# nemochina2008/soundgen_beta

Hardware: AMD Instinct MI355X
Metric: synthesized audio samples/sec (whole node) @44.1 kHz; RMS error vs R ref (higher is better)
Workload: dtype fp32 (fp64 phase)

## Files before the change

soundgen_beta_amd/csrc/sg_dev.h:

```cpp
#pragma once
#include <stdint.h>

struct SgSeg {
  double t0;
  double c0, c1, c2, c3, c4;
};

struct SgEpoch {
  int64_t w_off;
  int64_t amp_off;
  int64_t knot_off;
  int32_t seg_off;
  int32_t nseg;
  int32_t n;
  int32_t G;
  int32_t R;
  int32_t u0;
  double x1, xG;
  double xby;
  double invD;
  int32_t dj0, dj1;
  int64_t dk0;
  int32_t syl;
  int32_t pad;
// ... 125 lines not shown
  int32_t pad;
  int64_t chirp;
  int64_t bf;
};
struct SgFftGeom {
  SgCdft cd[2];
  int32_t wl, M, nstages, fb;
  int32_t radix[SG_FFT_MAX_STAGES];
  int64_t tw;
  int64_t win;
  int32_t lds_bytes;
  int32_t kind;
  uint32_t mr_magic[SG_FFT_MAX_STAGES], ns_magic[SG_FFT_MAX_STAGES];
  uint32_t m_magic, hp_magic;
  int64_t tws;
};

constexpr int SG_FFT_WG = 0;
constexpr int SG_FFT_WAVE = 1;
constexpr int SG_FFT_DFT = 2;
constexpr int SG_FFT_ODD = 3;
constexpr int SG_WAVE_STATE = 24;
constexpr int SG_FFT_WAVES = 8;

#ifndef SG_NOISE_WAVES
#define SG_NOISE_WAVES 12
#endif
constexpr int SG_FFT_WAVES_NOISE = SG_NOISE_WAVES;
constexpr int sg_fft_waves(int phase) { return phase == 0 ? SG_FFT_WAVES_NOISE : SG_FFT_WAVES; }
constexpr int SG_PF_SRC = 20;
constexpr int SG_PF_PAIR = 10;
// ... 161 lines not shown
```

soundgen_beta_amd/csrc/sg_exec.cpp:

```cpp
#include "sg_exec.h"
#include "sg_amp.h"
#include "sg_prof.h"

#include <algorithm>
#include <chrono>
#include <exception>
#include <thread>
#include <cmath>
#include <climits>
#include <atomic>
#include <map>
#include <cstdlib>
#include <cstdio>
#include <cstring>
#include <string>

namespace sg {

namespace {
#define HIPCHK(x)                                                                         \
  do {                                                                                    \
    hipError_t _e = (x);                                                                  \
    if (_e != hipSuccess)                                                                 \
      throw SgError(SG_E_DEVICE, std::string(#x) + ": " + hipGetErrorString(_e));     \
// ... 784 lines not shown
  DevicePlan& D0 = *runs[0].D;
  HIPCHK(hipEventRecord(D0.ev_fork, s));
  HIPCHK(hipStreamWaitEvent(s2, D0.ev_fork, 0));
  for (const PlanRun& r : runs) {
    device_execute_harm(*r.B, *r.D, r.out, s2, nullptr);
    HIPCHK(hipEventRecord(r.D->ev_join, s2));
  }
  for (const PlanRun& r : runs) device_execute_spec(*r.B, *r.D, r.out, s, nullptr, true, r.D->ev_join);
  HIPCHK(hipGetLastError());
}

void device_execute_spec(const Batch& B, const DevicePlan& D, float* d_out, hipStream_t s,
                         std::vector<SgProfEvent>* prof, bool join, hipEvent_t harm_done) {
  launch_spec_env(D, B, s);
  auto phase = [&](int ph) {
    const int64_t* r = B.fgroup_range[ph];
    const int64_t nseg = B.seg_range[ph][1] - B.seg_range[ph][0];
    hipEvent_t e0 = nullptr, e1 = nullptr;
    if (prof && nseg > 0) {
      HIPCHK(hipEventCreate(&e0));
      HIPCHK(hipEventCreate(&e1));
      HIPCHK(hipEventRecord(e0, s));
    }
    launch_stft_ola(D, ph, B.seg_range[ph][0], nseg, B.fgroup_lds[ph][0], s);
    if (prof && nseg > 0) {
      HIPCHK(hipEventRecord(e1, s));
      prof->push_back({SG_PROF_STFT_OLA, e0, e1});
    }
    launch_fft_frames(D, r[1], r[2] - r[1], B.fgroup_lds[ph][1], s);
    launch_fft_frames64(D, B, ph, s);
    const int64_t t0 = ph == 0 ? 0 : B.olatile_split, t1 = ph == 0 ? B.olatile_split : (int64_t)B.olatiles.size();
    const int64_t o0 = ph == 0 ? 0 : B.ola_split, o1 = ph == 0 ? B.ola_split : (int64_t)B.olas_dev.size();
    launch_ola(D, t0, t1 - t0, s);
    launch_ola_max(D, o0, o1 - o0, s);
  };
  phase(0);
  for (const Batch::Copy& c : B.copies)
    HIPCHK(hipMemcpyAsync(D.fs + c.fs_off, D.fl + c.fl_off, (size_t)c.n * sizeof(float), hipMemcpyDeviceToDevice, s));
  if (join) HIPCHK(hipStreamWaitEvent(s, harm_done, 0));
  launch_mix(D, 0, B.mixtile_hp, d_out, s);
  launch_mix_hp(D, B.mixtile_hp, B.mixtile_split - B.mixtile_hp, s);
  phase(1);
  launch_mix(D, B.mixtile_split, (int64_t)B.mixtiles.size() - B.mixtile_split, d_out, s);
  HIPCHK(hipGetLastError());
// ... 4 lines not shown
```

soundgen_beta_amd/csrc/sg_exec.h:

```cpp
#pragma once
#include <hip/hip_runtime.h>

#include <utility>
#include <vector>

#include "sg_plan.h"

namespace sg {

struct PcmJob {
  char* buf = nullptr;
  SgPcmCall* calls = nullptr;
  SgPcmTile* tiles = nullptr;
  SgPcmStat* stats = nullptr;
  int64_t n = 0, ntiles = 0;
  void prepare(const int64_t* off, const int64_t* len, int64_t n_calls, hipStream_t s);
  void run(const void* in, bool f64, int mode, double nrange, int16_t* out, hipStream_t s) const;
  void free();
};

struct DevicePlan {
  bool uploaded = false;
  char* arena = nullptr;
  size_t arena_bytes = 0;
// ... 88 lines not shown
void launch_ugather(const SgUJob* jobs, int64_t n_jobs, const float* us, float* fl, hipStream_t s);
void launch_sine_bank(const DevicePlan& D, int64_t k0, int64_t n, hipStream_t s);
void launch_sine_bank_pairs(const DevicePlan& D, int64_t k0, int64_t n, hipStream_t s);
void launch_sine_bank_tall(const DevicePlan& D, int64_t k0, int64_t n, hipStream_t s);
void launch_sine_bank_tall_pairs(const DevicePlan& D, int64_t k0, int64_t n, hipStream_t s);
void launch_syl_max(const DevicePlan& D, int64_t s0, int64_t n_syls, hipStream_t s);
void launch_piece_max(const DevicePlan& D, int64_t p0, int64_t n_ptiles, hipStream_t s);
void launch_harm_finalize(const DevicePlan& D, int64_t f0, int64_t n_stiles, float* out, hipStream_t s);
void launch_harm_copy(const DevicePlan& D, int64_t c0, int64_t n_ctiles, float* out, hipStream_t s);
void launch_sine_bank_hp(const DevicePlan& D, int64_t n, hipStream_t s);
void launch_sine_bank_tab(const DevicePlan& D, int logn, int64_t j0, int64_t n, float* out, hipStream_t s);
void launch_piece_max_hp(const DevicePlan& D, int64_t p0, int64_t n_ptiles, hipStream_t s);
void launch_harm_finalize_hp(const DevicePlan& D, int64_t n_stiles, hipStream_t s);
void launch_mix_hp(const DevicePlan& D, int64_t t0, int64_t n_tiles, hipStream_t s);
void launch_fft_frames64(const DevicePlan& D, const Batch& B, int ph, hipStream_t s);
void launch_fft_frames(const DevicePlan& D, int64_t g0, int64_t n_groups, int lds_bytes, hipStream_t s);
void launch_stft_ola(const DevicePlan& D, int phase, int64_t s0, int64_t n_segs, int lds_bytes, hipStream_t s);
void launch_ola(const DevicePlan& D, int64_t t0, int64_t n_tiles, hipStream_t s);
void launch_ola_max(const DevicePlan& D, int64_t o0, int64_t n_olas, hipStream_t s);
void launch_fft_probe(const SgFftGeom* geom, const float* fl, float* data, int M, int nframes, int inverse,
                      hipStream_t s);
void launch_mix(const DevicePlan& D, int64_t t0, int64_t n_tiles, float* out, hipStream_t s);
void launch_spec_env(const DevicePlan& D, const Batch& B, hipStream_t s);

}
```

soundgen_beta_amd/csrc/sg_fft.hip:

```cpp
#include <hip/hip_runtime.h>

#include <type_traits>

#include "sg_dev.h"
#include "sg_devfn.h"
#include "sg_fft64_dev.h"
#include "sg_roots.h"

namespace {

typedef float v2 __attribute__((ext_vector_type(2)));
__device__ __forceinline__ v2 V(float2 a) { return v2{a.x, a.y}; }
__device__ __forceinline__ float2 F(v2 a) { return make_float2(a.x, a.y); }
__device__ __forceinline__ v2 pfma(v2 a, v2 b, v2 c) { return __builtin_elementwise_fma(a, b, c); }
__device__ __forceinline__ v2 splat(float c) { return v2{c, c}; }
__device__ __forceinline__ v2 vmul(v2 a, v2 w) {
  v2 t, r;
  __asm__("v_pk_mul_f32 %0, %1, %2 op_sel_hi:[0,1]" : "=v"(t) : "v"(a), "v"(w));
  __asm__("v_pk_fma_f32 %0, %1, %2, %3 op_sel:[1,1,0] op_sel_hi:[1,0,1] neg_lo:[0,1,0]"
          : "=v"(r) : "v"(a), "v"(w), "v"(t));
  return r;
}
__device__ __forceinline__ v2 vmulc(v2 a, v2 w) {
  v2 t, r;
// ... 92 lines not shown

__device__ __forceinline__ void pack_pair(float2 yk, float2 ymk, float2 wNk, float2& zk, float2& zmk) {
  const float2 e = cadd(yk, cconj(ymk));
  const float2 d = csub(yk, cconj(ymk));
  const float2 o = cmulc(d, wNk);
  zk = make_float2(e.x - o.y, e.y + o.x);
  const float2 e2 = cadd(ymk, cconj(yk));
  const float2 d2 = csub(ymk, cconj(yk));
  const float2 o2 = make_float2(-(d2.x * wNk.x - d2.y * wNk.y), -(d2.x * wNk.y + d2.y * wNk.x));
  zmk = make_float2(e2.x - o2.y, e2.y + o2.x);
}

constexpr int SG_FFT_THREADS = 512;
constexpr int SG_FFT_SLOTS = 8192;

template <int R>
struct NbOf {
  static constexpr int value = (SG_FFT_SLOTS / SG_FFT_THREADS + R - 1) / R;
};

__device__ __forceinline__ int udiv(int n, uint32_t magic) {
  return magic ? (int)__umulhi((uint32_t)n, magic) : n;
}

template <int R, bool INV>
__device__ __forceinline__ void stage_ip(float2* X, int M, int Ns, const float2* twS, int fb, uint32_t mr_magic,
                                         uint32_t ns_magic) {
  constexpr int NB = NbOf<R>::value;
  constexpr bool ODD = (R % 2) == 1;
  constexpr int H = ODD ? (R - 1) / 2 : 1;
  const int MR = M / R;
  const int total = fb * MR;
  v2 st[NB][R];
  int base_o[NB];
  bool live[NB];
#pragma unroll
  for (int q = 0; q < NB; ++q) {
    const int idx = threadIdx.x + q * SG_FFT_THREADS;
    live[q] = idx < total;
    base_o[q] = 0;
    if (!live[q]) continue;
    const int f = udiv(idx, mr_magic);
    const int j = idx - f * MR;
    const float2* x = X + f * M;
    float2 v[R];
#pragma unroll
    for (int r = 0; r < R; ++r) v[r] = x[j + r * MR];
    const int jm = j - udiv(j, ns_magic) * Ns;
    if (Ns > 1) {
      const float2* tw = twS + (Ns - 1) + jm;
#pragma unroll
      for (int r = 1; r < R; ++r) {
        const float2 w = tw[(r - 1) * Ns];
// ... 27 lines not shown
#pragma unroll
      for (int k = 1; k <= H; ++k) {
        v2 a, b;
        odd_out<R, INV>(st[q], k, a, b);
        y[k * Ns] = F(a);
        y[(R - k) * Ns] = F(b);
      }
    } else {
#pragma unroll
      for (int r = 0; r < R; ++r) y[r * Ns] = F(st[q][r]);
    }
  }
  __syncthreads();
}

template <bool INV>
__device__ void fft_ip(float2* X, const SgFftGeom& g, const float2* twS, int fb) {
  int Ns = 1;
  for (int s = 0; s < g.nstages; ++s) {
    const int R = g.radix[s];
    const uint32_t mm = g.mr_magic[s], nm = g.ns_magic[s];
    int Ms = g.M;
    Ms = __builtin_amdgcn_readfirstlane(Ms);
    switch (R) {
#define SG_STAGE(RR) \
      case RR: stage_ip<RR, INV>(X, Ms, Ns, twS, fb, mm, nm); break;
      SG_STAGE(2) SG_STAGE(3) SG_STAGE(4) SG_STAGE(5) SG_STAGE(7) SG_STAGE(11) SG_STAGE(13) SG_STAGE(17)
      SG_STAGE(19) SG_STAGE(23) SG_STAGE(29) SG_STAGE(31)
#undef SG_STAGE
      default: break;
    }
    Ns *= R;
  }
}

__device__ __forceinline__ void sg_wave_fence() { __asm__ __volatile__("" ::: "memory"); }

template <int R>
struct NbW {
  static constexpr int value = SG_WAVE_STATE / R > 0 ? SG_WAVE_STATE / R : 1;
};

#ifndef SG_R19_REMAP
#define SG_R19_REMAP 1
#endif
template <int R, bool INV, int CM = 0, int CNS = 0>
__device__ __forceinline__ void stage_w(float2* X, int M_, int Ns_, const float2* twS, uint32_t ns_magic, int lane) {
  constexpr int NB = NbW<R>::value;
// ... 220 lines not shown
  }
  sg_wave_fence();
}

template <bool INV, int CM, int R0, int R1, int R2, bool MFMA = true, bool LAST = true>
__device__ __forceinline__ void fft_wc(float2* X, const float2* twS, const float4* A29, int lane SG_ST_PARAMS) {
  if constexpr (MFMA && CM == 1102 && R0 == 29) stage29_mfma<INV>(X, A29, lane);
  else stage_w<R0, INV, CM, 1>(X, CM, 1, twS, 0u, lane);
  SG_ST(INV ? 5 : 1);
  stage_w<R1, INV, CM, R0>(X, CM, R0, twS, 0u, lane);
  SG_ST(INV ? 6 : 2);
  if constexpr (LAST) stage_w<R2, INV, CM, R0 * R1>(X, CM, R0 * R1, twS, 0u, lane);
  SG_ST(INV ? 7 : 3);
}

template <bool INV>
__device__ void cdft(float2* X, const SgCdft& c, const SgFftGeom* __restrict__ geoms, const float* __restrict__ fl,
                     float2* Z, float2* tw) {
  const SgFftGeom& gs = geoms[c.geom];
  const int T = c.L ? c.L : c.n;
  const float2* twg = reinterpret_cast<const float2*>(fl + gs.tws);
  for (int t = threadIdx.x; t < T - 1; t += SG_FFT_THREADS) tw[t] = twg[t];
  if (!c.L) {
    __syncthreads();
    fft_ip<INV>(X, gs, tw, 1);
    return;
  }
  const int n = c.n, L = c.L;
  const float2* ch = reinterpret_cast<const float2*>(fl + c.chirp);
  const float2* bf = reinterpret_cast<const float2*>(fl + c.bf);
  for (int j = threadIdx.x; j < L; j += SG_FFT_THREADS)
    Z[j] = j < n ? cmul(INV ? cconj(X[j]) : X[j], ch[j]) : make_float2(0.f, 0.f);
  __syncthreads();
  fft_ip<false>(Z, gs, tw, 1);
  for (int k = threadIdx.x; k < L; k += SG_FFT_THREADS) Z[k] = cmul(Z[k], bf[k]);
  __syncthreads();
  fft_ip<true>(Z, gs, tw, 1);
  for (int k = threadIdx.x; k < n; k += SG_FFT_THREADS) {
    const float2 v = cmul(Z[k], ch[k]);
    X[k] = INV ? cconj(v) : v;
  }
  __syncthreads();
}

__device__ void odd_frame(const SgFrameGroup& G, const SgFrame* __restrict__ frames, const SgFftGeom& g,
                          const SgFftGeom* __restrict__ geoms, const float* __restrict__ fl, float* __restrict__ fs,
                          float4* lds4) {
  const int N = g.wl, M = g.M, N2 = 2 * M;
  const int T = max(g.cd[0].L ? g.cd[0].L : g.cd[0].n, g.cd[1].L ? g.cd[1].L : g.cd[1].n);
  float2* B = reinterpret_cast<float2*>(lds4);
  float2* Z = B + N;
  float2* tw = Z + T;
  const SgFrame F = frames[G.f0];
  const float* ham = fl + g.win;
  const float* han = ham + N;
  if (G.mode == SG_FRAME_FILTER) {
    const float* s = fs + F.src;
    for (int n = threadIdx.x; n < N; n += SG_FFT_THREADS) B[n] = make_float2(s[n] * ham[n], 0.f);
    __syncthreads();
    cdft<false>(B, g.cd[0], geoms, fl, Z, tw);
    const float* env = fl + F.env;
    const float invN = 1.f / (float)N;
    for (int k = threadIdx.x; k < M; k += SG_FFT_THREADS) {
      const float sc = invN * env[k];
      const float2 y = make_float2(B[k].x * sc, B[k].y * sc);
      B[k] = y;
      if (k > 0) B[N2 - k] = cconj(y);
      if (k == M - 1) B[M] = make_float2(y.x, 0.f);
    }
  } else {
    const float* u = fl + F.src;
    const float* flt = fl + F.env;
    for (int k = threadIdx.x; k < M; k += SG_FFT_THREADS) {
      const float2 y = make_float2(u[k] * flt[k], 0.f);
      B[k] = y;
      if (k > 0) B[N2 - k] = y;
      if (k == M - 1) B[M] = y;
    }
  }
  __syncthreads();
  cdft<true>(B, g.cd[1], geoms, fl, Z, tw);
  const float invN2 = 1.f / (float)N2;
  float* d = fs + F.dst;
  for (int i = threadIdx.x; i < N; i += SG_FFT_THREADS) d[i] = B[i < N2 ? i : i - N2].x * invN2 * han[i];
}

}

extern "C" __global__ __launch_bounds__(SG_FFT_THREADS) void sg_fft_frames(
    const SgFrameGroup* __restrict__ groups, const SgFrame* __restrict__ frames, const SgFftGeom* __restrict__ geoms,
    const float* __restrict__ fl, float* __restrict__ fs) {
  extern __shared__ float4 lds4[];
  float2* A = reinterpret_cast<float2*>(lds4);
  __shared__ SgFrame fr[16];
  const SgFrameGroup G = groups[blockIdx.x];
  const SgFftGeom& g = geoms[G.geom];
  if (g.kind == SG_FFT_ODD) {
    odd_frame(G, frames, g, geoms, fl, fs, lds4);
    return;
  }
  const int M = g.M, N = g.wl, fb = G.nf;
  const float2* twg = reinterpret_cast<const float2*>(fl + g.tw);
  const float2* twN = twg + M;
  float2* twM = A + fb * M;
  if (g.kind != SG_FFT_DFT) {
    const float2* tsg = reinterpret_cast<const float2*>(fl + g.tws);
    for (int t = threadIdx.x; t < M - 1; t += SG_FFT_THREADS) twM[t] = tsg[t];
  }
  if (threadIdx.x < fb) fr[threadIdx.x] = frames[G.f0 + threadIdx.x];
  __syncthreads();
  const float* ham = fl + g.win;
  const float* han = ham + N;
  const float invN = 1.f / (float)N;
  const int half = M / 2;
  const int npairs = fb * (half + 1);
  constexpr int NP = SG_FFT_SLOTS / 2 / SG_FFT_THREADS + 1;
  if (G.mode == SG_FRAME_FILTER) {
    for (int idx = threadIdx.x; idx < fb * M; idx += SG_FFT_THREADS) {
      const int f = udiv(idx, g.m_magic), n = idx - f * M;
      const float* s = fs + fr[f].src;
      A[idx] = make_float2(s[2 * n] * ham[2 * n], s[2 * n + 1] * ham[2 * n + 1]);
    }
    __syncthreads();
    if (g.kind == SG_FFT_DFT) cdft<false>(A, g.cd[0], geoms, fl, twM, twM + g.cd[0].L);
    else fft_ip<false>(A, g, twM, fb);
    float2 zk[NP], zm[NP], zh[NP];
    int pk[NP], pf[NP];
#pragma unroll
    for (int q = 0; q < NP; ++q) {
      const int idx = threadIdx.x + q * SG_FFT_THREADS;
      pk[q] = -1;
      if (idx >= npairs) continue;
      const int f = udiv(idx, g.hp_magic), k = idx - f * (half + 1);
      if (k != 0 && k >= M - k) continue;
      pk[q] = k;
      pf[q] = f;
      const float2* z = A + f * M;
      const float* env = fl + fr[f].env;
      auto X_at = [&](int kk) -> float2 {
        const float2 a = z[kk], b = z[(M - kk) % M];
        const float2 e = make_float2(0.5f * (a.x + b.x), 0.5f * (a.y - b.y));
        const float2 dd = make_float2(a.x - b.x, a.y + b.y);
        const float2 o = make_float2(0.5f * dd.y, -0.5f * dd.x);
        return cadd(e, cmul(o, twN[kk]));
      };
      if (k == 0) {
        const float2 x0 = X_at(0), xl = X_at(M - 1);
        const float y0 = x0.x * invN * env[0];
        const float nyq = xl.x * invN * env[M - 1];
        zk[q] = make_float2(y0 + nyq, y0 - nyq);
        if (M % 2 == 0) {
          const float2 xk = X_at(half);
          const float2 yk = make_float2(xk.x * invN * env[half], xk.y * invN * env[half]);
// ... 10 lines not shown
    __syncthreads();
#pragma unroll
    for (int q = 0; q < NP; ++q) {
      if (pk[q] < 0) continue;
      float2* out = A + pf[q] * M;
      const int k = pk[q];
      out[k] = zk[q];
      if (k == 0) {
        if (M % 2 == 0) out[half] = zh[q];
      } else {
        out[M - k] = zm[q];
      }
    }
    __syncthreads();
  } else {
    for (int idx = threadIdx.x; idx < npairs; idx += SG_FFT_THREADS) {
      const int f = udiv(idx, g.hp_magic), k = idx - f * (half + 1);
      const SgFrame& F = fr[f];
      const float* u = fl + F.src;
      const float* flt = fl + F.env;
      float2* out = A + f * M;
      if (k == 0) {
        const float y0 = u[0] * flt[0], nyq = u[M - 1] * flt[M - 1];
        out[0] = make_float2(y0 + nyq, y0 - nyq);
        if (M % 2 == 0) {
          const float2 yk = make_float2(u[half] * flt[half], 0.f);
          float2 a, b;
          pack_pair(yk, yk, twN[half], a, b);
          out[half] = a;
        }
      } else if (k < M - k) {
        const float2 yk = make_float2(u[k] * flt[k], 0.f), ym = make_float2(u[M - k] * flt[M - k], 0.f);
        float2 a, b;
        pack_pair(yk, ym, twN[k], a, b);
        out[k] = a;
        out[M - k] = b;
      }
    }
    __syncthreads();
  }
  if (g.kind == SG_FFT_DFT) cdft<true>(A, g.cd[0], geoms, fl, twM, twM + g.cd[0].L);
  else fft_ip<true>(A, g, twM, fb);
  for (int idx = threadIdx.x; idx < fb * M; idx += SG_FFT_THREADS) {
    const int f = udiv(idx, g.m_magic), n = idx - f * M;
    const float2 v = A[idx];
    float* d = fs + fr[f].dst;
    d[2 * n] = v.x * invN * han[2 * n];
    d[2 * n + 1] = v.y * invN * han[2 * n + 1];
  }
}

static_assert(SG_PF_PAIR <= SG_PF_SRC, "noise filter pairs alias the sound pairs");
struct FramePf {
  float2 s[SG_PF_SRC];
  float2 a[SG_PF_PAIR];
  float xh, xh2;
  __device__ __forceinline__ float2& b(int i) { return s[i]; }
  __device__ __forceinline__ const float2& b(int i) const { return s[i]; }
};

template <bool FUSED = false>
__device__ __forceinline__ void frame_prefetch(FramePf& P, const SgFrame& F, int mode, int M,
                                               const float* __restrict__ fl, const float* __restrict__ fs, int lane) {
  const int half = M / 2;
// ... 1037 lines not shown
  } while (0)

static void lds_opt_in(const void* fn, int lds_bytes, const char* name) {
  static std::mutex mu;
  static std::map<std::pair<const void*, int>, int> done;
  int dev = 0;
  if (hipGetDevice(&dev) != hipSuccess) throw SgError(SG_E_DEVICE, std::string(name) + ": hipGetDevice failed");
  std::lock_guard<std::mutex> lk(mu);
  int& have = done[{fn, dev}];
  if (lds_bytes <= have) return;
  if (hipFuncSetAttribute(fn, hipFuncAttributeMaxDynamicSharedMemorySize, lds_bytes) != hipSuccess)
    throw SgError(SG_E_DEVICE, std::string(name) + ": dynamic LDS " + std::to_string(lds_bytes) + " B refused");
  have = lds_bytes;
}

void launch_fft_frames(const DevicePlan& D, int64_t g0, int64_t n_groups, int lds_bytes, hipStream_t s) {
  if (n_groups <= 0) return;
  lds_opt_in(reinterpret_cast<const void*>(&sg_fft_frames), lds_bytes, "sg_fft_frames");
  hipLaunchKernelGGL(sg_fft_frames, dim3((unsigned)n_groups), dim3(SG_FFT_THREADS), lds_bytes, s, D.fgroups + g0,
                     D.frames,
                     D.geoms, D.fl, D.fs);
  SG_LAUNCHED("sg_fft_frames");
}
void launch_stft_ola(const DevicePlan& D, int phase, int64_t s0, int64_t n_segs, int lds_bytes, hipStream_t s) {
  if (n_segs <= 0) return;
  auto* k = phase == 0 ? &sg_stft_ola_noise : &sg_stft_ola;
  lds_opt_in(reinterpret_cast<const void*>(k), lds_bytes, phase == 0 ? "sg_stft_ola_noise" : "sg_stft_ola");
  const int W = sg_fft_waves(phase);
  if (n_segs % W) throw SgError(SG_E_DEVICE, "sg_stft_ola: segment count not a multiple of the workgroup's waves");
  hipLaunchKernelGGL(k, dim3((unsigned)(n_segs / W)), dim3(W * 64), lds_bytes, s,
                     D.olasegs + s0,
                     D.olas, D.frames, D.geoms, D.fl, D.fs, D.olatilemax);
  SG_LAUNCHED("sg_stft_ola");
}
void launch_fft_probe(const SgFftGeom* geom, const float* fl, float* data, int M, int nframes, int inverse,
                      hipStream_t s) {
// ... 70 lines not shown
```

soundgen_beta_amd/csrc/sg_plan.h:

```cpp
#pragma once
#include <cstdint>
#include <functional>
#include <memory>
#include <utility>
#include <vector>

#include "sg_dev.h"
#include "sg_rmath.h"
#include "soundgen_hip.h"

namespace sg {

template <class T>
struct NoInitAlloc : std::allocator<T> {
  template <class U>
  struct rebind { using other = NoInitAlloc<U>; };
  NoInitAlloc() = default;
  template <class U>
  NoInitAlloc(const NoInitAlloc<U>&) noexcept {}
  T* allocate(size_t n) {
    if (n * sizeof(T) < SG_BULK_HUGE) return std::allocator<T>::allocate(n);
    return static_cast<T*>(bulk_alloc(n * sizeof(T)));
  }
  void deallocate(T* p, size_t n) noexcept {
// ... 75 lines not shown
  std::vector<SgOla> olas[2];
  std::vector<SgFrame64> frames64;
  std::vector<int32_t> roots64_wl;
  std::vector<int64_t> roots64_off, frames64_tab;
  int64_t roots64_total = 0;
  int32_t frames64_maxwl = 0;
  int64_t frames64_noise = 0;
  int64_t frames64_w[2] = {0, 0};
  std::vector<SgNoiseItem> items;
  std::vector<SgMix> mixes[2];
  struct Copy { int64_t fl_off, fs_off, n; };
  std::vector<Copy> copies;
  std::vector<SgFrameGroup> fgroups;
  int64_t fgroup_range[2][3] = {{0, 0, 0}, {0, 0, 0}};
  int fgroup_lds[2][2] = {{0, 0}, {0, 0}};
  std::vector<SgOla> olas_dev;
  std::vector<SgOlaTile> olatiles;
  int64_t olatile_split = 0, ola_split = 0;
  std::vector<SgSegment> olasegs;
  int32_t n_segslots = 0;
  int64_t seg_range[2][2] = {{0, 0}, {0, 0}};
  std::vector<SgMix> mixes_dev;
  std::vector<SgMixTile> mixtiles;
  int64_t mixtile_split = 0;
  int64_t mixtile_hp = 0;
  bulk<double> cknots;
  int64_t w_total = 0;
  int64_t w64_total = 0;
  int64_t fh_total = 0;
  int64_t hp_bouts = 0;
// ... 91 lines not shown
```

soundgen_beta_amd/csrc/sg_plan_spec.cpp:

```cpp
#include <algorithm>
#include <atomic>
#include <cmath>
#include <complex>
#include <cstdio>
#include <cstdlib>
#include <cstring>
#include <map>
#include <memory>
#include <mutex>
#include <string>

#include "sg_plan.h"
#include "sg_prof.h"

#ifndef SG_SEG_SORT
#define SG_SEG_SORT 1
#endif
#ifndef SG_ENV_SORT
#define SG_ENV_SORT 1
#endif

namespace sg {

namespace {
// ... 115 lines not shown
      b[m] = std::complex<double>((*ch)[2 * m], -(*ch)[2 * m + 1]);
      if (m > 0) b[L - m] = b[m];
    }
    dft_smooth(b, bf);
    vec v(2 * (size_t)L);
    for (int k = 0; k < L; ++k) {
      v[2 * k] = bf[k].real() / L;
      v[2 * k + 1] = bf[k].imag() / L;
    }
    return v;
  });
  c.chirp = fl_push(B, ch->data(), (int64_t)ch->size());
  c.bf = fl_push(B, bv->data(), (int64_t)bv->size());
  return c;
}
static int cdft_size(const SgCdft& c) { return c.L ? c.L : c.n; }

static int geometry_odd(Batch& B, int wl) {
  SgFftGeom g{};
  g.wl = wl;
  g.M = wl / 2;
  g.kind = SG_FFT_ODD;
  g.fb = 1;
  g.cd[0] = make_cdft(B, wl);
  g.cd[1] = make_cdft(B, 2 * g.M);
  const int T = std::max(cdft_size(g.cd[0]), cdft_size(g.cd[1]));
  g.lds_bytes = (int32_t)(((int64_t)wl + 2 * (int64_t)T) * 8);
  if (g.lds_bytes > 160 * 1024) throw SgError(SG_E_UNSUPPORTED, "FFT: odd window length exceeds the LDS budget");
  g.win = push_windows(B, wl);
  for (size_t i = 0; i < B.geoms.size(); ++i)
    if (B.geoms[i].wl == wl) return (int)i;
  B.geoms.push_back(g);
  return (int)B.geoms.size() - 1;
}

int geometry(Batch& B, int wl) {
  for (size_t i = 0; i < B.geoms.size(); ++i)
    if (B.geoms[i].wl == wl) return (int)i;
  if (wl < 3) throw SgError(SG_E_UNSUPPORTED, "FFT: window length must be >= 3");
  if (wl % 2) return geometry_odd(B, wl);
  SgFftGeom g{};
  g.wl = wl;
  g.M = wl / 2;
  int m = g.M;
  for (int r : kRadices) {
    while (m % r == 0) {
      if (g.nstages >= SG_FFT_MAX_STAGES) throw SgError(SG_E_UNSUPPORTED, "FFT: too many stages");
      g.radix[g.nstages++] = r;
      m /= r;
    }
  }
  const bool dft = m != 1;
  if (dft) {
    g.nstages = 0;
    g.cd[0] = make_cdft(B, g.M);
    for (size_t i = 0; i < B.geoms.size(); ++i)
      if (B.geoms[i].wl == wl) return (int)i;
  }
  const int M = g.M;
  const auto tw = trig_table(1, wl, [M, wl] {
    vec w(4 * (size_t)M);
    for (int t = 0; t < M; ++t) {
      const double a = -2.0 * M_PI * (double)t / (double)M;
      w[2 * t] = std::cos(a);
      w[2 * t + 1] = std::sin(a);
      const double b = -2.0 * M_PI * (double)t / (double)wl;
      w[2 * M + 2 * t] = std::cos(b);
      w[2 * M + 2 * t + 1] = std::sin(b);
    }
    return w;
// ... 20 lines not shown
    g.tws = fl_push(B, ts->data(), (int64_t)ts->size());
  }
  g.win = push_windows(B, wl);
  g.kind = dft ? SG_FFT_DFT : SG_FFT_WAVE;
  for (int s = 0; s < g.nstages && !dft; ++s) {
    const int r = g.radix[s], nb = (g.M / r + 63) / 64;
    if (nb > std::max(1, SG_WAVE_STATE / r)) g.kind = SG_FFT_WG;
  }
  if (!dft && (g.M > 64 * SG_PF_SRC || g.M / 2 + 1 > 64 * SG_PF_PAIR)) g.kind = SG_FFT_WG;
  if (!dft && (int64_t)(SG_FFT_WAVES + 4) * g.M * 8 > 160 * 1024) g.kind = SG_FFT_WG;
  if (g.kind == SG_FFT_WAVE) {
    g.fb = SG_FFT_WAVES;
    g.lds_bytes = (SG_FFT_WAVES + 4) * g.M * 8;
  } else if (g.kind == SG_FFT_DFT) {
    g.fb = 1;
    g.lds_bytes = (g.M + 2 * g.cd[0].L) * 8;
    if (g.lds_bytes > 160 * 1024) throw SgError(SG_E_UNSUPPORTED, "FFT: Bluestein frame exceeds the LDS budget");
  } else {
    g.fb = std::max(1, std::min(16, kFftSlots / g.M));
    if (g.fb * g.M > kFftSlots) throw SgError(SG_E_UNSUPPORTED, "FFT: window too long for LDS (wl > 16384)");
    g.lds_bytes = (g.fb + 1) * g.M * 8;
  }
  auto magic = [](int d) -> uint32_t { return d <= 1 ? 0u : (uint32_t)(((1ull << 32) + (uint64_t)d - 1) / (uint64_t)d); };
  int ns = 1;
  for (int s = 0; s < g.nstages; ++s) {
    g.mr_magic[s] = magic(g.M / g.radix[s]);
    g.ns_magic[s] = magic(ns);
    ns *= g.radix[s];
  }
  g.m_magic = magic(g.M);
  g.hp_magic = magic(g.M / 2 + 1);
// ... 551 lines not shown
      for (size_t w = i; w < i + 4 && w < B.envtasks.size(); ++w) { mx = std::max(mx, cost(B.envtasks[w])); wsum += cost(B.envtasks[w]); }
      wmax += 4 * mx;
    }
    std::fprintf(stderr, "sg plan: envelope tasks %zu, workgroup cost %.3g, used %.3g (%.1f%% idle)\n", B.envtasks.size(), wmax,
                 wsum, wmax > 0 ? 100.0 * (wmax - wsum) / wmax : 0.0);
  }
  B.fgroups.clear();
  std::vector<int64_t> pos[2];
  for (int ph = 0; ph < 2; ++ph) {
    const size_t ng = B.geoms.size();
    std::vector<int64_t> rank(ng), start(ng + 1, 0);
    {
      std::vector<int32_t> og(ng);
      for (size_t g = 0; g < ng; ++g) og[g] = (int32_t)g;
      std::stable_sort(og.begin(), og.end(), [&](int32_t a, int32_t b) {
        const int ka = B.geoms[a].kind == SG_FFT_WAVE ? 0 : 1, kb = B.geoms[b].kind == SG_FFT_WAVE ? 0 : 1;
        return ka != kb ? ka < kb : a < b;
      });
      for (size_t r = 0; r < ng; ++r) rank[og[r]] = (int64_t)r;
    }
    for (int32_t gi : B.frame_geom[ph]) ++start[rank[gi] + 1];
    for (size_t r = 0; r < ng; ++r) start[r + 1] += start[r];
    std::vector<int64_t> idx(B.frames[ph].size());
    for (size_t i = 0; i < idx.size(); ++i) idx[start[rank[B.frame_geom[ph][i]]]++] = (int64_t)i;
    std::vector<SgFrame> fr(idx.size());
    std::vector<int32_t> fg(idx.size());
    pos[ph].assign(idx.size(), 0);
    for (size_t i = 0; i < idx.size(); ++i) {
      fr[i] = B.frames[ph][idx[i]];
      fg[i] = B.frame_geom[ph][idx[i]];
      pos[ph][idx[i]] = (int64_t)i;
    }
    B.frames[ph] = fr;
    B.frame_geom[ph] = fg;
    const int32_t base = ph == 0 ? 0 : (int32_t)B.frames[0].size();
    B.fgroup_lds[ph][0] = B.fgroup_lds[ph][1] = 0;
    B.fgroup_range[ph][0] = B.fgroup_range[ph][1] = (int64_t)B.fgroups.size();
    for (size_t i = 0; i < fr.size();) {
      const int gi = fg[i];
      const SgFftGeom& g = B.geoms[gi];
      if (g.kind == SG_FFT_WAVE) {
        B.fgroup_lds[ph][0] = std::max(B.fgroup_lds[ph][0], (sg_fft_waves(ph) + 4) * g.M * 8 + (g.M == 1102 ? 2048 : 0));
        ++i;
        continue;
      }
      size_t j = i;
      while (j < fr.size() && fg[j] == gi && (int)(j - i) < g.fb) ++j;
      B.fgroups.push_back(SgFrameGroup{gi, ph == 0 ? SG_FRAME_NOISE : SG_FRAME_FILTER, base + (int32_t)i,
                                       (int32_t)(j - i)});
      B.fgroup_lds[ph][1] = std::max(B.fgroup_lds[ph][1], g.lds_bytes);
      i = j;
    }
    B.fgroup_range[ph][2] = (int64_t)B.fgroups.size();
  }
  B.olas_dev.clear();
  B.olatiles.clear();
  B.olasegs.clear();
  B.ola_split = (int64_t)B.olas[0].size();
  for (int ph = 0; ph < 2; ++ph) {
    if (ph == 1) B.olatile_split = (int64_t)B.olatiles.size();
    const int32_t base = ph == 0 ? 0 : (int32_t)B.frames[0].size();
    for (const SgOla& o0 : B.olas[ph]) {
// ... 146 lines not shown
    for (const auto& kv : gfr) gs.push_back({kv.second, kv.first});
    std::sort(gs.rbegin(), gs.rend());
    for (size_t i = 0; i < gs.size() && i < 16; ++i) {
      const SgFftGeom& g = B.geoms[gs[i].second];
      std::string rs;
      for (int s = 0; s < g.nstages; ++s) rs += (s ? "x" : "") + std::to_string(g.radix[s]);
      std::fprintf(stderr, "sg plan: geom wl=%d M=%d radices %s: %lld frames\n", g.wl, g.M, rs.c_str(),
                   (long long)gs[i].first);
    }
    std::map<int32_t, int64_t> gun;
    for (const SgFrameGroup& fg : B.fgroups) gun[fg.geom] += fg.nf;
    for (const auto& kv : gun) {
      const SgFftGeom& g = B.geoms[kv.first];
      std::string rs;
      for (int s = 0; s < g.nstages; ++s) rs += (s ? "x" : "") + std::to_string(g.radix[s]);
      std::fprintf(stderr, "sg plan: unfused geom wl=%d M=%d kind %d radices %s: %lld frames\n", g.wl, g.M, g.kind,
                   rs.c_str(), (long long)kv.second);
    }
    std::fprintf(stderr, "sg plan: %lld fused segments (%lld slots incl. padding), %lld frames owned, %lld computed (%.1f%% recomputed)\n",
                 (long long)real, (long long)B.olasegs.size(), (long long)owned, (long long)run,
                 owned ? 100.0 * (double)(run - owned) / (double)owned : 0.0);
  }
  for (SgNoiseItem& it : B.items)
    if (it.flags & SG_ITEM_FILTER_OLA) {
      it.ola += (int32_t)B.ola_split;
      it.flags &= ~SG_ITEM_FILTER_OLA;
    }
  B.mixes_dev.clear();
  B.mixtiles.clear();
  for (int pass = 0; pass < 3; ++pass) {
    const int ph = pass == 2 ? 1 : 0;
    if (pass == 1) B.mixtile_hp = (int64_t)B.mixtiles.size();
    if (pass == 2) B.mixtile_split = (int64_t)B.mixtiles.size();
// ... 19 lines not shown
```

Before: 14.06 billion.

## Add specialized small-radix FFT frame kernel with reduced LDS and per-class launches

Adds a sg_fft_frames_small kernel variant for Bluestein/odd-length FFT geometries whose stages use only radix 2-5. It compiles out the large-radix stages, reads twiddles directly from global memory instead of staging them in LDS, and handles one frame per group. Frame groups are sorted and split into classes by kernel type and LDS size bucket, and each class gets its own launch sized to its own LDS need. The goal is lower register and LDS use and therefore higher occupancy for these frames. The costs are extra kernel launches and twiddle reads that now go to global memory instead of LDS.

After: 14.05 billion. Within noise of the previous version (-0.1%).

```diff
diff --git a/soundgen_beta_amd/csrc/sg_dev.h b/soundgen_beta_amd/csrc/sg_dev.h
--- a/soundgen_beta_amd/csrc/sg_dev.h
+++ b/soundgen_beta_amd/csrc/sg_dev.h
@@ -163,7 +163,17 @@
   uint32_t mr_magic[SG_FFT_MAX_STAGES], ns_magic[SG_FFT_MAX_STAGES];
   uint32_t m_magic, hp_magic;
   int64_t tws;
-};
+  int32_t small;
+  int32_t pad;
+};
+
+constexpr int SG_FFT_LDS_CLASSES = 3;
+constexpr int sg_fft_lds_class(int lds_bytes) { return lds_bytes <= 53 * 1024 ? 0 : lds_bytes <= 80 * 1024 ? 1 : 2; }
+constexpr int SG_FRAMES_GENERAL = 0;
+constexpr int SG_FRAMES_SMALL = 1;
+#ifndef SG_SMALL_TW_LDS
+#define SG_SMALL_TW_LDS 0
+#endif
 
 constexpr int SG_FFT_WG = 0;
 constexpr int SG_FFT_WAVE = 1;
diff --git a/soundgen_beta_amd/csrc/sg_exec.cpp b/soundgen_beta_amd/csrc/sg_exec.cpp
--- a/soundgen_beta_amd/csrc/sg_exec.cpp
+++ b/soundgen_beta_amd/csrc/sg_exec.cpp
@@ -822,7 +822,6 @@
                          std::vector<SgProfEvent>* prof, bool join, hipEvent_t harm_done) {
   launch_spec_env(D, B, s);
   auto phase = [&](int ph) {
-    const int64_t* r = B.fgroup_range[ph];
     const int64_t nseg = B.seg_range[ph][1] - B.seg_range[ph][0];
     hipEvent_t e0 = nullptr, e1 = nullptr;
     if (prof && nseg > 0) {
@@ -835,7 +834,7 @@
       HIPCHK(hipEventRecord(e1, s));
       prof->push_back({SG_PROF_STFT_OLA, e0, e1});
     }
-    launch_fft_frames(D, r[1], r[2] - r[1], B.fgroup_lds[ph][1], s);
+    for (const Batch::FrameClass& fc : B.fclasses[ph]) launch_fft_frames(D, fc.g0, fc.n, fc.lds, fc.kernel, s);
     launch_fft_frames64(D, B, ph, s);
     const int64_t t0 = ph == 0 ? 0 : B.olatile_split, t1 = ph == 0 ? B.olatile_split : (int64_t)B.olatiles.size();
     const int64_t o0 = ph == 0 ? 0 : B.ola_split, o1 = ph == 0 ? B.ola_split : (int64_t)B.olas_dev.size();
diff --git a/soundgen_beta_amd/csrc/sg_exec.h b/soundgen_beta_amd/csrc/sg_exec.h
--- a/soundgen_beta_amd/csrc/sg_exec.h
+++ b/soundgen_beta_amd/csrc/sg_exec.h
@@ -126,7 +126,7 @@
 void launch_harm_finalize_hp(const DevicePlan& D, int64_t n_stiles, hipStream_t s);
 void launch_mix_hp(const DevicePlan& D, int64_t t0, int64_t n_tiles, hipStream_t s);
 void launch_fft_frames64(const DevicePlan& D, const Batch& B, int ph, hipStream_t s);
-void launch_fft_frames(const DevicePlan& D, int64_t g0, int64_t n_groups, int lds_bytes, hipStream_t s);
+void launch_fft_frames(const DevicePlan& D, int64_t g0, int64_t n_groups, int lds_bytes, int kernel, hipStream_t s);
 void launch_stft_ola(const DevicePlan& D, int phase, int64_t s0, int64_t n_segs, int lds_bytes, hipStream_t s);
 void launch_ola(const DevicePlan& D, int64_t t0, int64_t n_tiles, hipStream_t s);
 void launch_ola_max(const DevicePlan& D, int64_t o0, int64_t n_olas, hipStream_t s);
diff --git a/soundgen_beta_amd/csrc/sg_fft.hip b/soundgen_beta_amd/csrc/sg_fft.hip
--- a/soundgen_beta_amd/csrc/sg_fft.hip
+++ b/soundgen_beta_amd/csrc/sg_fft.hip
@@ -130,19 +130,19 @@
 constexpr int SG_FFT_THREADS = 512;
 constexpr int SG_FFT_SLOTS = 8192;
 
-template <int R>
+template <int R, int THREADS = SG_FFT_THREADS, int SLOTS = SG_FFT_SLOTS>
 struct NbOf {
-  static constexpr int value = (SG_FFT_SLOTS / SG_FFT_THREADS + R - 1) / R;
+  static constexpr int value = (SLOTS / THREADS + R - 1) / R;
 };
 
 __device__ __forceinline__ int udiv(int n, uint32_t magic) {
   return magic ? (int)__umulhi((uint32_t)n, magic) : n;
 }
 
-template <int R, bool INV>
+template <int R, bool INV, int THREADS, int SLOTS>
 __device__ __forceinline__ void stage_ip(float2* X, int M, int Ns, const float2* twS, int fb, uint32_t mr_magic,
                                          uint32_t ns_magic) {
-  constexpr int NB = NbOf<R>::value;
+  constexpr int NB = NbOf<R, THREADS, SLOTS>::value;
   constexpr bool ODD = (R % 2) == 1;
   constexpr int H = ODD ? (R - 1) / 2 : 1;
   const int MR = M / R;
@@ -152,7 +152,7 @@
   bool live[NB];
 #pragma unroll
   for (int q = 0; q < NB; ++q) {
-    const int idx = threadIdx.x + q * SG_FFT_THREADS;
+    const int idx = threadIdx.x + q * THREADS;
     live[q] = idx < total;
     base_o[q] = 0;
     if (!live[q]) continue;
@@ -210,8 +210,8 @@
   __syncthreads();
 }
 
-template <bool INV>
-__device__ void fft_ip(float2* X, const SgFftGeom& g, const float2* twS, int fb) {
+template <bool INV, bool SMALL = false, int THREADS = SG_FFT_THREADS, int SLOTS = SG_FFT_SLOTS>
+__device__ __forceinline__ void fft_ip_body(float2* X, const SgFftGeom& g, const float2* twS, int fb) {
   int Ns = 1;
   for (int s = 0; s < g.nstages; ++s) {
     const int R = g.radix[s];
@@ -220,14 +220,25 @@
     Ms = __builtin_amdgcn_readfirstlane(Ms);
     switch (R) {
 #define SG_STAGE(RR) \
-      case RR: stage_ip<RR, INV>(X, Ms, Ns, twS, fb, mm, nm); break;
-      SG_STAGE(2) SG_STAGE(3) SG_STAGE(4) SG_STAGE(5) SG_STAGE(7) SG_STAGE(11) SG_STAGE(13) SG_STAGE(17)
-      SG_STAGE(19) SG_STAGE(23) SG_STAGE(29) SG_STAGE(31)
+      case RR: stage_ip<RR, INV, THREADS, SLOTS>(X, Ms, Ns, twS, fb, mm, nm); break;
+#define SG_STAGE_BIG(RR) \
+      case RR: if constexpr (!SMALL) stage_ip<RR, INV, THREADS, SLOTS>(X, Ms, Ns, twS, fb, mm, nm); break;
+      SG_STAGE(2) SG_STAGE(3) SG_STAGE(4) SG_STAGE(5) SG_STAGE_BIG(7) SG_STAGE_BIG(11) SG_STAGE_BIG(13)
+      SG_STAGE_BIG(17) SG_STAGE_BIG(19) SG_STAGE_BIG(23) SG_STAGE_BIG(29) SG_STAGE_BIG(31)
 #undef SG_STAGE
+#undef SG_STAGE_BIG
       default: break;
     }
     Ns *= R;
   }
+}
+template <bool INV, bool SMALL = false, int THREADS = SG_FFT_THREADS, int SLOTS = SG_FFT_SLOTS>
+__device__ void fft_ip(float2* X, const SgFftGeom& g, const float2* twS, int fb) {
+  fft_ip_body<INV, SMALL, THREADS, SLOTS>(X, g, twS, fb);
+}
+template <bool INV, int THREADS, int SLOTS>
+__device__ __forceinline__ void fft_ip_small(float2* X, const SgFftGeom& g, const float2* twS) {
+  fft_ip_body<INV, true, THREADS, SLOTS>(X, g, twS, 1);
 }
 
 __device__ __forceinline__ void sg_wave_fence() { __asm__ __volatile__("" ::: "memory"); }
@@ -478,36 +489,54 @@
   SG_ST(INV ? 7 : 3);
 }
 
-template <bool INV>
-__device__ void cdft(float2* X, const SgCdft& c, const SgFftGeom* __restrict__ geoms, const float* __restrict__ fl,
+template <bool INV, bool SMALL = false, int THREADS = SG_FFT_THREADS, int SLOTS = SG_FFT_SLOTS>
+__device__ __forceinline__ void cdft_body(float2* X, const SgCdft& c, const SgFftGeom* __restrict__ geoms, const float* __restrict__ fl,
                      float2* Z, float2* tw) {
   const SgFftGeom& gs = geoms[c.geom];
   const int T = c.L ? c.L : c.n;
   const float2* twg = reinterpret_cast<const float2*>(fl + gs.tws);
-  for (int t = threadIdx.x; t < T - 1; t += SG_FFT_THREADS) tw[t] = twg[t];
+  if constexpr (SMALL && !SG_SMALL_TW_LDS) tw = const_cast<float2*>(twg);
+  else
+    for (int t = threadIdx.x; t < T - 1; t += THREADS) tw[t] = twg[t];
   if (!c.L) {
     __syncthreads();
-    fft_ip<INV>(X, gs, tw, 1);
+    if constexpr (SMALL) fft_ip_small<INV, THREADS, SLOTS>(X, gs, tw);
+    else fft_ip<INV, SMALL, THREADS, SLOTS>(X, gs, tw, 1);
     return;
   }
   const int n = c.n, L = c.L;
   const float2* ch = reinterpret_cast<const float2*>(fl + c.chirp);
   const float2* bf = reinterpret_cast<const float2*>(fl + c.bf);
-  for (int j = threadIdx.x; j < L; j += SG_FFT_THREADS)
+  for (int j = threadIdx.x; j < L; j += THREADS)
     Z[j] = j < n ? cmul(INV ? cconj(X[j]) : X[j], ch[j]) : make_float2(0.f, 0.f);
   __syncthreads();
-  fft_ip<false>(Z, gs, tw, 1);
-  for (int k = threadIdx.x; k < L; k += SG_FFT_THREADS) Z[k] = cmul(Z[k], bf[k]);
+  if constexpr (SMALL) fft_ip_small<false, THREADS, SLOTS>(Z, gs, tw);
+  else fft_ip<false, SMALL, THREADS, SLOTS>(Z, gs, tw, 1);
+  for (int k = threadIdx.x; k < L; k += THREADS) Z[k] = cmul(Z[k], bf[k]);
   __syncthreads();
-  fft_ip<true>(Z, gs, tw, 1);
-  for (int k = threadIdx.x; k < n; k += SG_FFT_THREADS) {
+  if constexpr (SMALL) fft_ip_small<true, THREADS, SLOTS>(Z, gs, tw);
+  else fft_ip<true, SMALL, THREADS, SLOTS>(Z, gs, tw, 1);
+  for (int k = threadIdx.x; k < n; k += THREADS) {
     const float2 v = cmul(Z[k], ch[k]);
     X[k] = INV ? cconj(v) : v;
   }
   __syncthreads();
 }
 
-__device__ void odd_frame(const SgFrameGroup& G, const SgFrame* __restrict__ frames, const SgFftGeom& g,
+template <bool INV, bool SMALL = false, int THREADS = SG_FFT_THREADS, int SLOTS = SG_FFT_SLOTS>
+__device__ void cdft(float2* X, const SgCdft& c, const SgFftGeom* __restrict__ geoms, const float* __restrict__ fl,
+                     float2* Z, float2* tw) {
+  if constexpr (SMALL) cdft_body<INV, true, THREADS, SLOTS>(X, c, geoms, fl, Z, tw);
+  else cdft_body<INV>(X, c, geoms, fl, Z, tw);
+}
+template <bool INV, int THREADS, int SLOTS>
+__device__ __forceinline__ void cdft_small(float2* X, const SgCdft& c, const SgFftGeom* __restrict__ geoms,
+                                           const float* __restrict__ fl, float2* Z, float2* tw) {
+  cdft_body<INV, true, THREADS, SLOTS>(X, c, geoms, fl, Z, tw);
+}
+
+template <bool SMALL = false, int THREADS = SG_FFT_THREADS, int SLOTS = SG_FFT_SLOTS>
+__device__ __forceinline__ void odd_frame_body(const SgFrameGroup& G, const SgFrame* __restrict__ frames, const SgFftGeom& g,
                           const SgFftGeom* __restrict__ geoms, const float* __restrict__ fl, float* __restrict__ fs,
                           float4* lds4) {
   const int N = g.wl, M = g.M, N2 = 2 * M;
@@ -520,12 +549,13 @@
   const float* han = ham + N;
   if (G.mode == SG_FRAME_FILTER) {
     const float* s = fs + F.src;
-    for (int n = threadIdx.x; n < N; n += SG_FFT_THREADS) B[n] = make_float2(s[n] * ham[n], 0.f);
+    for (int n = threadIdx.x; n < N; n += THREADS) B[n] = make_float2(s[n] * ham[n], 0.f);
     __syncthreads();
-    cdft<false>(B, g.cd[0], geoms, fl, Z, tw);
+    if constexpr (SMALL) cdft_small<false, THREADS, SLOTS>(B, g.cd[0], geoms, fl, Z, tw);
+    else cdft<false>(B, g.cd[0], geoms, fl, Z, tw);
     const float* env = fl + F.env;
     const float invN = 1.f / (float)N;
-    for (int k = threadIdx.x; k < M; k += SG_FFT_THREADS) {
+    for (int k = threadIdx.x; k < M; k += THREADS) {
       const float sc = invN * env[k];
       const float2 y = make_float2(B[k].x * sc, B[k].y * sc);
       B[k] = y;
@@ -535,7 +565,7 @@
   } else {
     const float* u = fl + F.src;
     const float* flt = fl + F.env;
-    for (int k = threadIdx.x; k < M; k += SG_FFT_THREADS) {
+    for (int k = threadIdx.x; k < M; k += THREADS) {
       const float2 y = make_float2(u[k] * flt[k], 0.f);
       B[k] = y;
       if (k > 0) B[N2 - k] = y;
@@ -543,64 +573,81 @@
     }
   }
   __syncthreads();
-  cdft<true>(B, g.cd[1], geoms, fl, Z, tw);
+  if constexpr (SMALL) cdft_small<true, THREADS, SLOTS>(B, g.cd[1], geoms, fl, Z, tw);
+  else cdft<true>(B, g.cd[1], geoms, fl, Z, tw);
   const float invN2 = 1.f / (float)N2;
   float* d = fs + F.dst;
-  for (int i = threadIdx.x; i < N; i += SG_FFT_THREADS) d[i] = B[i < N2 ? i : i - N2].x * invN2 * han[i];
-}
-
-}
-
-extern "C" __global__ __launch_bounds__(SG_FFT_THREADS) void sg_fft_frames(
-    const SgFrameGroup* __restrict__ groups, const SgFrame* __restrict__ frames, const SgFftGeom* __restrict__ geoms,
-    const float* __restrict__ fl, float* __restrict__ fs) {
-  extern __shared__ float4 lds4[];
+  for (int i = threadIdx.x; i < N; i += THREADS) d[i] = B[i < N2 ? i : i - N2].x * invN2 * han[i];
+}
+
+__device__ void odd_frame(const SgFrameGroup& G, const SgFrame* __restrict__ frames, const SgFftGeom& g,
+                          const SgFftGeom* __restrict__ geoms, const float* __restrict__ fl, float* __restrict__ fs,
+                          float4* lds4) {
+  odd_frame_body<>(G, frames, g, geoms, fl, fs, lds4);
+}
+
+template <bool SMALL, int THREADS, int SLOTS>
+__device__ __forceinline__ void frames_body(const SgFrameGroup* __restrict__ groups,
+                                            const SgFrame* __restrict__ frames,
+                                            const SgFftGeom* __restrict__ geoms, const float* __restrict__ fl,
+                                            float* __restrict__ fs, float4* lds4, SgFrame* fr) {
   float2* A = reinterpret_cast<float2*>(lds4);
-  __shared__ SgFrame fr[16];
   const SgFrameGroup G = groups[blockIdx.x];
   const SgFftGeom& g = geoms[G.geom];
   if (g.kind == SG_FFT_ODD) {
-    odd_frame(G, frames, g, geoms, fl, fs, lds4);
+    if constexpr (SMALL) odd_frame_body<true, THREADS, SLOTS>(G, frames, g, geoms, fl, fs, lds4);
+    else odd_frame(G, frames, g, geoms, fl, fs, lds4);
     return;
   }
-  const int M = g.M, N = g.wl, fb = G.nf;
+  const int M = g.M, N = g.wl, fb = SMALL ? 1 : G.nf;
   const float2* twg = reinterpret_cast<const float2*>(fl + g.tw);
   const float2* twN = twg + M;
   float2* twM = A + fb * M;
-  if (g.kind != SG_FFT_DFT) {
-    const float2* tsg = reinterpret_cast<const float2*>(fl + g.tws);
-    for (int t = threadIdx.x; t < M - 1; t += SG_FFT_THREADS) twM[t] = tsg[t];
-  }
-  if (threadIdx.x < fb) fr[threadIdx.x] = frames[G.f0 + threadIdx.x];
-  __syncthreads();
+  SgFrame F1{};
+  if constexpr (SMALL) {
+    F1 = frames[G.f0];
+  } else {
+    if (g.kind != SG_FFT_DFT) {
+      const float2* tsg = reinterpret_cast<const float2*>(fl + g.tws);
+      for (int t = threadIdx.x; t < M - 1; t += THREADS) twM[t] = tsg[t];
+    }
+    if (threadIdx.x < fb) fr[threadIdx.x] = frames[G.f0 + threadIdx.x];
+    __syncthreads();
+  }
+  auto frame_of = [&](int f) -> const SgFrame& {
+    if constexpr (SMALL) return F1;
+    else return fr[f];
+  };
+  auto frame_idx = [&](int idx, uint32_t magic) -> int { return SMALL ? 0 : udiv(idx, magic); };
   const float* ham = fl + g.win;
   const float* han = ham + N;
   const float invN = 1.f / (float)N;
   const int half = M / 2;
   const int npairs = fb * (half + 1);
-  constexpr int NP = SG_FFT_SLOTS / 2 / SG_FFT_THREADS + 1;
+  constexpr int NP = (SMALL ? SLOTS / 4 : SLOTS / 2) / THREADS + 1;
   if (G.mode == SG_FRAME_FILTER) {
-    for (int idx = threadIdx.x; idx < fb * M; idx += SG_FFT_THREADS) {
-      const int f = udiv(idx, g.m_magic), n = idx - f * M;
-      const float* s = fs + fr[f].src;
+    for (int idx = threadIdx.x; idx < fb * M; idx += THREADS) {
+      const int f = frame_idx(idx, g.m_magic), n = idx - f * M;
+      const float* s = fs + frame_of(f).src;
       A[idx] = make_float2(s[2 * n] * ham[2 * n], s[2 * n + 1] * ham[2 * n + 1]);
     }
     __syncthreads();
-    if (g.kind == SG_FFT_DFT) cdft<false>(A, g.cd[0], geoms, fl, twM, twM + g.cd[0].L);
+    if constexpr (SMALL) cdft_small<false, THREADS, SLOTS>(A, g.cd[0], geoms, fl, twM, twM + g.cd[0].L);
+    else if (g.kind == SG_FFT_DFT) cdft<false>(A, g.cd[0], geoms, fl, twM, twM + g.cd[0].L);
     else fft_ip<false>(A, g, twM, fb);
     float2 zk[NP], zm[NP], zh[NP];
     int pk[NP], pf[NP];
 #pragma unroll
     for (int q = 0; q < NP; ++q) {
-      const int idx = threadIdx.x + q * SG_FFT_THREADS;
+      const int idx = threadIdx.x + q * THREADS;
       pk[q] = -1;
       if (idx >= npairs) continue;
-      const int f = udiv(idx, g.hp_magic), k = idx - f * (half + 1);
+      const int f = frame_idx(idx, g.hp_magic), k = idx - f * (half + 1);
       if (k != 0 && k >= M - k) continue;
       pk[q] = k;
       pf[q] = f;
       const float2* z = A + f * M;
-      const float* env = fl + fr[f].env;
+      const float* env = fl + frame_of(f).env;
       auto X_at = [&](int kk) -> float2 {
         const float2 a = z[kk], b = z[(M - kk) % M];
         const float2 e = make_float2(0.5f * (a.x + b.x), 0.5f * (a.y - b.y));
@@ -641,9 +688,9 @@
     }
     __syncthreads();
   } else {
-    for (int idx = threadIdx.x; idx < npairs; idx += SG_FFT_THREADS) {
-      const int f = udiv(idx, g.hp_magic), k = idx - f * (half + 1);
-      const SgFrame& F = fr[f];
+    for (int idx = threadIdx.x; idx < npairs; idx += THREADS) {
+      const int f = frame_idx(idx, g.hp_magic), k = idx - f * (half + 1);
+      const SgFrame& F = frame_of(f);
       const float* u = fl + F.src;
       const float* flt = fl + F.env;
       float2* out = A + f * M;
@@ -666,15 +713,33 @@
     }
     __syncthreads();
   }
-  if (g.kind == SG_FFT_DFT) cdft<true>(A, g.cd[0], geoms, fl, twM, twM + g.cd[0].L);
+  if constexpr (SMALL) cdft_small<true, THREADS, SLOTS>(A, g.cd[0], geoms, fl, twM, twM + g.cd[0].L);
+  else if (g.kind == SG_FFT_DFT) cdft<true>(A, g.cd[0], geoms, fl, twM, twM + g.cd[0].L);
   else fft_ip<true>(A, g, twM, fb);
-  for (int idx = threadIdx.x; idx < fb * M; idx += SG_FFT_THREADS) {
-    const int f = udiv(idx, g.m_magic), n = idx - f * M;
+  for (int idx = threadIdx.x; idx < fb * M; idx += THREADS) {
+    const int f = frame_idx(idx, g.m_magic), n = idx - f * M;
     const float2 v = A[idx];
-    float* d = fs + fr[f].dst;
+    float* d = fs + frame_of(f).dst;
     d[2 * n] = v.x * invN * han[2 * n];
     d[2 * n + 1] = v.y * invN * han[2 * n + 1];
   }
+}
+
+}
+
+extern "C" __global__ __launch_bounds__(SG_FFT_THREADS) void sg_fft_frames(
+    const SgFrameGroup* __restrict__ groups, const SgFrame* __restrict__ frames, const SgFftGeom* __restrict__ geoms,
+    const float* __restrict__ fl, float* __restrict__ fs) {
+  extern __shared__ float4 lds4[];
+  __shared__ SgFrame fr[16];
+  frames_body<false, SG_FFT_THREADS, SG_FFT_SLOTS>(groups, frames, geoms, fl, fs, lds4, fr);
+}
+
+extern "C" __global__ __launch_bounds__(SG_FFT_THREADS) __attribute__((amdgpu_waves_per_eu(4))) void sg_fft_frames_small(
+    const SgFrameGroup* __restrict__ groups, const SgFrame* __restrict__ frames, const SgFftGeom* __restrict__ geoms,
+    const float* __restrict__ fl, float* __restrict__ fs) {
+  extern __shared__ float4 lds4[];
+  frames_body<true, SG_FFT_THREADS, SG_FFT_SLOTS>(groups, frames, geoms, fl, fs, lds4, nullptr);
 }
 
 static_assert(SG_PF_PAIR <= SG_PF_SRC, "noise filter pairs alias the sound pairs");
@@ -1742,12 +1807,12 @@
   have = lds_bytes;
 }
 
-void launch_fft_frames(const DevicePlan& D, int64_t g0, int64_t n_groups, int lds_bytes, hipStream_t s) {
+void launch_fft_frames(const DevicePlan& D, int64_t g0, int64_t n_groups, int lds_bytes, int kernel, hipStream_t s) {
   if (n_groups <= 0) return;
-  lds_opt_in(reinterpret_cast<const void*>(&sg_fft_frames), lds_bytes, "sg_fft_frames");
-  hipLaunchKernelGGL(sg_fft_frames, dim3((unsigned)n_groups), dim3(SG_FFT_THREADS), lds_bytes, s, D.fgroups + g0,
-                     D.frames,
-                     D.geoms, D.fl, D.fs);
+  auto* k = kernel == SG_FRAMES_SMALL ? &sg_fft_frames_small : &sg_fft_frames;
+  lds_opt_in(reinterpret_cast<const void*>(k), lds_bytes, kernel == SG_FRAMES_SMALL ? "sg_fft_frames_small" : "sg_fft_frames");
+  hipLaunchKernelGGL(k, dim3((unsigned)n_groups), dim3(SG_FFT_THREADS), lds_bytes, s, D.fgroups + g0, D.frames, D.geoms, D.fl,
+                     D.fs);
   SG_LAUNCHED("sg_fft_frames");
 }
 void launch_stft_ola(const DevicePlan& D, int phase, int64_t s0, int64_t n_segs, int lds_bytes, hipStream_t s) {
diff --git a/soundgen_beta_amd/csrc/sg_plan.h b/soundgen_beta_amd/csrc/sg_plan.h
--- a/soundgen_beta_amd/csrc/sg_plan.h
+++ b/soundgen_beta_amd/csrc/sg_plan.h
@@ -113,6 +113,8 @@
   std::vector<SgFrameGroup> fgroups;
   int64_t fgroup_range[2][3] = {{0, 0, 0}, {0, 0, 0}};
   int fgroup_lds[2][2] = {{0, 0}, {0, 0}};
+  struct FrameClass { int64_t g0, n; int lds, kernel; };
+  std::vector<FrameClass> fclasses[2];
   std::vector<SgOla> olas_dev;
   std::vector<SgOlaTile> olatiles;
   int64_t olatile_split = 0, ola_split = 0;
diff --git a/soundgen_beta_amd/csrc/sg_plan_spec.cpp b/soundgen_beta_amd/csrc/sg_plan_spec.cpp
--- a/soundgen_beta_amd/csrc/sg_plan_spec.cpp
+++ b/soundgen_beta_amd/csrc/sg_plan_spec.cpp
@@ -153,7 +153,17 @@
   c.bf = fl_push(B, bv->data(), (int64_t)bv->size());
   return c;
 }
+static int frame_class_key(const SgFftGeom& g) {
+  if (g.kind == SG_FFT_WAVE) return 0;
+  return g.small ? 2 + sg_fft_lds_class(g.lds_bytes) : 1;
+}
 static int cdft_size(const SgCdft& c) { return c.L ? c.L : c.n; }
+static bool cdft_small(const Batch& B, const SgCdft& c) {
+  const SgFftGeom& g = B.geoms[c.geom];
+  for (int s = 0; s < g.nstages; ++s)
+    if (g.radix[s] > 5) return false;
+  return true;
+}
 
 static int geometry_odd(Batch& B, int wl) {
   SgFftGeom g{};
@@ -163,8 +173,10 @@
   g.fb = 1;
   g.cd[0] = make_cdft(B, wl);
   g.cd[1] = make_cdft(B, 2 * g.M);
+  g.small = cdft_small(B, g.cd[0]) && cdft_small(B, g.cd[1]);
   const int T = std::max(cdft_size(g.cd[0]), cdft_size(g.cd[1]));
-  g.lds_bytes = (int32_t)(((int64_t)wl + 2 * (int64_t)T) * 8);
+  const int twl = g.small && !SG_SMALL_TW_LDS ? 1 : 2;
+  g.lds_bytes = (int32_t)(((int64_t)wl + twl * (int64_t)T) * 8);
   if (g.lds_bytes > 160 * 1024) throw SgError(SG_E_UNSUPPORTED, "FFT: odd window length exceeds the LDS budget");
   g.win = push_windows(B, wl);
   for (size_t i = 0; i < B.geoms.size(); ++i)
@@ -193,6 +205,7 @@
   if (dft) {
     g.nstages = 0;
     g.cd[0] = make_cdft(B, g.M);
+    g.small = cdft_small(B, g.cd[0]);
     for (size_t i = 0; i < B.geoms.size(); ++i)
       if (B.geoms[i].wl == wl) return (int)i;
   }
@@ -243,7 +256,7 @@
     g.lds_bytes = (SG_FFT_WAVES + 4) * g.M * 8;
   } else if (g.kind == SG_FFT_DFT) {
     g.fb = 1;
-    g.lds_bytes = (g.M + 2 * g.cd[0].L) * 8;
+    g.lds_bytes = (g.M + (g.small && !SG_SMALL_TW_LDS ? 1 : 2) * g.cd[0].L) * 8;
     if (g.lds_bytes > 160 * 1024) throw SgError(SG_E_UNSUPPORTED, "FFT: Bluestein frame exceeds the LDS budget");
   } else {
     g.fb = std::max(1, std::min(16, kFftSlots / g.M));
@@ -825,7 +838,7 @@
       std::vector<int32_t> og(ng);
       for (size_t g = 0; g < ng; ++g) og[g] = (int32_t)g;
       std::stable_sort(og.begin(), og.end(), [&](int32_t a, int32_t b) {
-        const int ka = B.geoms[a].kind == SG_FFT_WAVE ? 0 : 1, kb = B.geoms[b].kind == SG_FFT_WAVE ? 0 : 1;
+        const int ka = frame_class_key(B.geoms[a]), kb = frame_class_key(B.geoms[b]);
         return ka != kb ? ka < kb : a < b;
       });
       for (size_t r = 0; r < ng; ++r) rank[og[r]] = (int64_t)r;
@@ -847,6 +860,8 @@
     const int32_t base = ph == 0 ? 0 : (int32_t)B.frames[0].size();
     B.fgroup_lds[ph][0] = B.fgroup_lds[ph][1] = 0;
     B.fgroup_range[ph][0] = B.fgroup_range[ph][1] = (int64_t)B.fgroups.size();
+    B.fclasses[ph].clear();
+    int last_key = 0;
     for (size_t i = 0; i < fr.size();) {
       const int gi = fg[i];
       const SgFftGeom& g = B.geoms[gi];
@@ -857,6 +872,14 @@
       }
       size_t j = i;
       while (j < fr.size() && fg[j] == gi && (int)(j - i) < g.fb) ++j;
+      if (const int key = frame_class_key(g); key != last_key) {
+        B.fclasses[ph].push_back(
+            Batch::FrameClass{(int64_t)B.fgroups.size(), 0, 0, g.small ? SG_FRAMES_SMALL : SG_FRAMES_GENERAL});
+        last_key = key;
+      }
+      Batch::FrameClass& fc = B.fclasses[ph].back();
+      ++fc.n;
+      fc.lds = std::max(fc.lds, g.lds_bytes);
       B.fgroups.push_back(SgFrameGroup{gi, ph == 0 ? SG_FRAME_NOISE : SG_FRAME_FILTER, base + (int32_t)i,
                                        (int32_t)(j - i)});
       B.fgroup_lds[ph][1] = std::max(B.fgroup_lds[ph][1], g.lds_bytes);
@@ -1033,9 +1056,13 @@
       const SgFftGeom& g = B.geoms[kv.first];
       std::string rs;
       for (int s = 0; s < g.nstages; ++s) rs += (s ? "x" : "") + std::to_string(g.radix[s]);
-      std::fprintf(stderr, "sg plan: unfused geom wl=%d M=%d kind %d radices %s: %lld frames\n", g.wl, g.M, g.kind,
-                   rs.c_str(), (long long)kv.second);
-    }
+      std::fprintf(stderr, "sg plan: unfused geom wl=%d M=%d kind %d small %d lds %d radices %s: %lld frames\n", g.wl, g.M,
+                   g.kind, g.small, g.lds_bytes, rs.c_str(), (long long)kv.second);
+    }
+    for (int ph = 0; ph < 2; ++ph)
+      for (const Batch::FrameClass& fc : B.fclasses[ph])
+        std::fprintf(stderr, "sg plan: phase %d: unfused class kernel %d: %lld groups, %d B of LDS\n", ph, fc.kernel,
+                     (long long)fc.n, fc.lds);
     std::fprintf(stderr, "sg plan: %lld fused segments (%lld slots incl. padding), %lld frames owned, %lld computed (%.1f%% recomputed)\n",
                  (long long)real, (long long)B.olasegs.size(), (long long)owned, (long long)run,
                  owned ? 100.0 * (double)(run - owned) / (double)owned : 0.0);
```
